# RohitMovva/VexAutonomousPlanner

Measured on AMD Instinct MI355X. Metric: trajectory sample-points/sec (batched paths), higher is better.
Workload: dtype f32; 1 GPU; c3: 4096 paths x 32 waypoints x 10000 samples per GPU; waypoints=32, samples=10000, recurrence=f64 behind fp32 rows, parallelism=paths sharded x1, no data-path collective

## Files before the change

vexautonomousplanner_amd/csrc/vap_sample.hip:

```cpp
#include "vap_device.h"
#include "vap_kernels.h"

#include <cstdio>
#include <cstdlib>
#include <type_traits>
#include <vector>

namespace vap {

static_assert(kCoefBlockDoubles == kCoefDoubles, "scratch sizing and block layout disagree");
static_assert(kGridRunBlockDoubles == kGridRunDoubles, "scratch sizing and run-table layout disagree");

template <typename OT, bool COEF_LDS, bool HI, int PPB = 1>
__global__ __launch_bounds__(kSampleThreads, 3) void k_sample(int B, int W, int S, int tile, int tiles_per_block,
                                                           const double *__restrict__ power,
                                                           const double *__restrict__ seg_rows,
                                                           const double *__restrict__ lut,
                                                           const double *__restrict__ slopes,
                                                           const double *__restrict__ meta,
                                                           const double *__restrict__ aux,
                                                           const double *__restrict__ runs,
                                                           OT *__restrict__ ox, OT *__restrict__ oy,
                                                           OT *__restrict__ oh, OT *__restrict__ ok,
                                                           OT *__restrict__ odth, double *__restrict__ ok64,
                                                           double *__restrict__ odth64, long long *__restrict__ stats)
{
    static_assert(!HI || sizeof(OT) == 4, "the fp64 side rows belong to the fp32 output mode");
    extern __shared__ __attribute__((aligned(16))) double s_coef[];
    __shared__ double sD_all[PPB * kLutN], sWt_all[PPB * kLutN];
    __shared__ double s_dx[2][kSampleThreads], s_dy[2][kSampleThreads];
    __shared__ int s_j[2][kSampleThreads];
    __shared__ OT s_th[2][kSampleThreads];
    const long long ts0 = stats ? __builtin_amdgcn_s_memtime() : 0;
    const int tid = threadIdx.x;
    const int G = W - 1;
    const int tile0 = blockIdx.x * tiles_per_block;
    if (tile0 * tile >= S) return;
    const bool writer = tile == kSampleChunk || tid < kSampleThreads - 1;
    constexpr int VW = 16 / sizeof(OT);
    const bool aligned = (S % VW) == 0;

    int p_b[PPB], p_N[PPB], p_nruns[PPB];
    bool p_live[PPB];
    double p_tmax[PPB], p_total[PPB], p_dd[PPB], p_lstep[PPB], p_tstep[PPB], p_inv[PPB], p_sk[PPB];
    double run_touch = 0.0;
#pragma unroll
    for (int pp = 0; pp < PPB; pp++) {
        const int bq = blockIdx.y * PPB + pp;
        p_live[pp] = bq < B;
        const int b = p_live[pp] ? bq : B - 1;
        p_b[pp] = b;
        const double *m = meta + (size_t)b * kMetaStride;
        p_tmax[pp] = m[0]; p_total[pp] = m[1]; p_dd[pp] = m[2];
        p_N[pp] = (int)m[3];
        const double *ax = aux + (size_t)b * kAuxStride;
        p_lstep[pp] = ax[0]; p_tstep[pp] = ax[1]; p_inv[pp] = ax[2];
        p_nruns[pp] = (int)ax[3];
        run_touch += runs[(size_t)b * kGridRunDoubles + (tid < 120 ? tid : 0)];
    }
    __shared__ double s_end[PPB][2];
    double end_d1x = 1.0, end_d1y = 1.0;
    {
        const int pp = tid < PPB ? tid : 0;
        if (seg_rows && tid < PPB && p_live[pp]) {
            end_d1x = seg_rows[((size_t)p_b[pp] * G + (G - 1)) * 12 + 6];
            end_d1y = seg_rows[((size_t)p_b[pp] * G + (G - 1)) * 12 + 7];
        }
    }
    {
        constexpr int ITER = 4;
        double vD[PPB][ITER], vW[PPB][ITER];
#pragma unroll
        for (int pp = 0; pp < PPB; pp++) {
            const bool go = p_live[pp];
#pragma unroll
            for (int it = 0; it < ITER; it++) {
                const int i = tid + it * kSampleThreads;
                vD[pp][it] = (go && i < kLutN) ? lut[(size_t)p_b[pp] * kLutN + i] : 0.0;
                vW[pp][it] = (go && slopes && i < kLutN) ? slopes[(size_t)p_b[pp] * kLutN + i] : 0.0;
            }
        }
        static_assert(ITER * kSampleThreads >= kLutN, "one pass covers the table");
#pragma unroll
        for (int pp = 0; pp < PPB; pp++) {
            if (tid == pp) {
                double rx = 1.0, ry = 1.0;
                if (fabs(end_d1x) <= 1e-9 * fabs(end_d1y) || fabs(end_d1y) <= 1e-9 * fabs(end_d1x))
                    hermite_eval_ref(seg_rows + (size_t)p_b[pp] * G * 12, p_tmax[pp], G, 1, (double)(W - 1), rx, ry);
                s_end[pp][0] = fabs(rx) <= 1e-12 * fabs(ry) ? rx : __builtin_nan("");
                s_end[pp][1] = fabs(ry) <= 1e-12 * fabs(rx) ? ry : __builtin_nan("");
            }
        }
        if constexpr (COEF_LDS) {
#pragma unroll
            for (int pp = 0; pp < PPB; pp++)
                if (p_live[pp])
                    lds_fill<4>(s_coef + (size_t)pp * G * kCoefDoubles, power + (size_t)p_b[pp] * G * kCoefDoubles, G * kCoefDoubles, tid,
                                kSampleThreads);
        }
#pragma unroll
        for (int pp = 0; pp < PPB; pp++) {
#pragma unroll
            for (int it = 0; it < ITER; it++) {
                const int i = tid + it * kSampleThreads;
                if (i < kLutN) {
                    sD_all[pp * kLutN + i] = vD[pp][it];
                    if (slopes) sWt_all[pp * kLutN + i] = vW[pp][it];
                }
            }
        }
    }
    auto grid_first_of = [&](const double *run_tab, double dd, int N, int n_runs, int kb0) {
        const int dd_exp = (__double2hiint(dd) >> 20) & 0x7ff;
        const int kf = kb0 < N - 1 ? kb0 : N - 1;
        int r = 2 + 2 * (((__double2hiint((double)kf * dd) >> 20) & 0x7ff) - dd_exp);
        r = kf <= 0 ? 0 : r < 1 ? 1 : r;
        r = r > n_runs - 1 ? n_runs - 1 : r;
        const double *e = run_tab + 3 * r;
        int ka = (int)grid_run_k0(e, 0);
        const int kb = (int)grid_run_k0(e, 1);
        double sa = e[1], da = e[2];
        if (kf < ka || kf >= kb) {
            while ((int)grid_run_k0(run_tab, r + 1) <= kf) r++;
            while (r > 0 && (int)grid_run_k0(run_tab, r) > kf) r--;
            ka = (int)grid_run_k0(run_tab, r);
            sa = run_tab[3 * r + 1];
            da = run_tab[3 * r + 2];
        }
        return sa + (double)(kf - ka) * da;
    };
#pragma unroll
    for (int pp = 0; pp < PPB; pp++)
        p_sk[pp] = (p_live[pp] && tile0 * tile < p_N[pp])
                       ? grid_first_of(runs + (size_t)p_b[pp] * kGridRunDoubles, p_dd[pp], p_N[pp], p_nruns[pp], tile0 * tile + tid * kSPT)
                       : 0.0;
    constexpr bool kSlopeOnDemand = PPB == 2;
    if (!slopes && !kSlopeOnDemand) {
        __syncthreads();
#pragma unroll
        for (int pp = 0; pp < PPB; pp++) {
            if (p_live[pp] && tile0 * tile < p_N[pp]) {
                const double *sDp = sD_all + pp * kLutN;
                for (int j = tid; j < kLutN; j += kSampleThreads) {
                    double w = 0.0;
                    if (j > 0) {
                        const double t0 = (double)(j - 1) * p_lstep[pp], t1 = (j == kLutN - 1) ? p_tmax[pp] : (double)j * p_lstep[pp];
                        w = div_inrange(t1 - t0, sDp[j] - sDp[j - 1]);
                    }
                    sWt_all[pp * kLutN + j] = w;
                }
            }
        }
    }
    __syncthreads();
    asm volatile("" ::"v"(run_touch));
    const long long ts1 = stats ? __builtin_amdgcn_s_memtime() : 0;
    const double end_param = (double)(W - 1);
    const int tab_n = W * kSamplesPerNode;
    int tiles_done = 0;

#pragma unroll 1
    for (int pp = 0; pp < PPB; pp++) {
    const int bq = blockIdx.y * PPB + pp;
    if (bq >= B) break;
    const int b = bq;
    const double *m = meta + (size_t)b * kMetaStride;
    const double t_max = m[0], total = m[1], dd = m[2];
    const int N = (int)m[3];
    const double *ax = aux + (size_t)b * kAuxStride;
    const double lstep = ax[0], tstep = ax[1], inv_tstep = ax[2];
    const int n_runs = (int)ax[3];
    const size_t row = (size_t)b * S;
    const double *sD = sD_all + pp * kLutN, *sWt = sWt_all + pp * kLutN;
    const double *pw = power + (size_t)b * G * kCoefDoubles;
    const double *coef = COEF_LDS ? s_coef + (size_t)pp * G * kCoefDoubles : pw;
    const double *run_tab = runs + (size_t)b * kGridRunDoubles;
    const double sk_first = PPB == 1 ? p_sk[0] : (pp == 0 ? p_sk[0] : p_sk[PPB - 1]);
    auto grid_first = [&](int kb0) { return grid_first_of(run_tab, dd, N, n_runs, kb0); };
    for (int tl = 0; tl < tiles_per_block; tl++) {
        const int k0 = (tile0 + tl) * tile;
        if (k0 >= S) break;
        const int kbase = k0 + tid * kSPT;
        auto store_vec = [&](OT *dst, const OT v[kSPT]) {
            if (!dst || !writer) return;
            if (aligned && kbase + kSPT <= S) {
                if constexpr (sizeof(OT) == 4) {
                    if constexpr (HI) {
                        using f4 = float __attribute__((ext_vector_type(4)));
                        f4 w = {v[0], v[1], v[2], v[3]};
                        __builtin_nontemporal_store(w, reinterpret_cast<f4 *>(dst + row + kbase));
                    } else {
                        *reinterpret_cast<float4 *>(dst + row + kbase) = make_float4(v[0], v[1], v[2], v[3]);
                    }
                } else {
                    *reinterpret_cast<double2 *>(dst + row + kbase) = make_double2(v[0], v[1]);
                    *reinterpret_cast<double2 *>(dst + row + kbase + 2) = make_double2(v[2], v[3]);
                }
            } else {
#pragma unroll
                for (int i = 0; i < kSPT; i++)
                    if (kbase + i < S) dst[row + kbase + i] = v[i];
            }
        };
        auto store_hi = [&](double *dst, const double v[kSPT]) {
            if (!writer) return;
            if ((S & 1) == 0 && kbase + kSPT <= S) {
                *reinterpret_cast<double2 *>(dst + row + kbase) = make_double2(v[0], v[1]);
                *reinterpret_cast<double2 *>(dst + row + kbase + 2) = make_double2(v[2], v[3]);
            } else {
#pragma unroll
                for (int i = 0; i < kSPT; i++)
                    if (kbase + i < S) dst[row + kbase + i] = v[i];
            }
        };
        if (k0 >= N) {
            const OT z[kSPT] = {(OT)0, (OT)0, (OT)0, (OT)0};
            store_vec(ox, z); store_vec(oy, z); store_vec(oh, z); store_vec(ok, z); store_vec(odth, z);
            if constexpr (HI) {
                const double zd[kSPT] = {0.0, 0.0, 0.0, 0.0};
                store_hi(ok64, zd); store_hi(odth64, zd);
            }
            continue;
        }
        auto tile_body = [&](auto interior_tag) {
            constexpr bool INTERIOR = decltype(interior_tag)::value;
        OT vx[kSPT], vy[kSPT], vh[kSPT], vk[kSPT], vd[kSPT];
        double vd64[HI ? kSPT : 1];
        [[maybe_unused]] double kap_even = 0.0;
        double sk = tl == 0 ? sk_first : grid_first(kbase);
        double d1x[kSPT], d1y[kSPT];
        int jjv[kSPT];
        int idx = 0;
        double tA[kSPT], sA[kSPT];
        int idxA[kSPT];
        bool redo[kSPT], any_redo = false;
        bool walk_on[kSPT], any_walk = false;
#pragma unroll
        for (int i = 0; i < kSPT; i++) {
            const int k = INTERIOR ? kbase + i : (kbase + i < N - 1 ? kbase + i : N - 1);
            if (i > 0) sk = sk + dd;
            const double s = INTERIOR ? sk : ((k == N - 1) ? total : sk);
            walk_on[i] = false;
            if (i == 0) {
                idx = lut_search_left_fixed(sD, s);
                if constexpr (!INTERIOR) idx = idx < 1 ? 1 : idx;
            } else {
                const int i1 = idx + 1 < kLutN - 1 ? idx + 1 : kLutN - 1;
                const double a0 = sD[idx], a1 = sD[i1];
                const bool st1 = idx < kLutN - 1 && a0 < s;
                const bool st2 = st1 && idx + 1 < kLutN - 1 && a1 < s;
                idx += (int)st1 + (int)st2;
                walk_on[i] = st2;
                any_walk |= st2;
            }
            sA[i] = s;
            idxA[i] = idx;
        }
        if (__builtin_expect(any_walk, 0)) {
#pragma unroll
            for (int i = 1; i < kSPT; i++) {
                if (walk_on[i]) {
                    int ix = idxA[i];
                    while (ix < kLutN - 1 && sD[ix] < sA[i]) ix++;
                    idxA[i] = ix;
                }
            }
        }
#pragma unroll
        for (int i = 0; i < kSPT; i++) {
            const double s = sA[i];
            const int idx = idxA[i];
            const double d0 = sD[idx - 1];
            const double t0 = (double)(idx - 1) * lstep;
            const bool exact = INTERIOR ? false : (s <= 0.0 || s >= total);
            double wslope;
            if (kSlopeOnDemand && !slopes) {
                const double t1 = (idx == kLutN - 1) ? t_max : (double)idx * lstep;
                wslope = div_inrange(t1 - t0, sD[idx] - d0);
            } else {
                wslope = sWt[idx];
            }
            double t = fma(wslope, s - d0, t0);
            if constexpr (!INTERIOR) t = s >= total ? end_param : t;
            bool near;
            jjv[i] = table_index_fast(t, tab_n, inv_tstep, near);
            tA[i] = t;
            redo[i] = near && !exact;
            any_redo |= redo[i];
        }
        if (__builtin_expect(any_redo, 0)) {
#pragma unroll
            for (int i = 0; i < kSPT; i++) {
                if (redo[i]) {
                    const int ix = idxA[i];
                    const double d0 = sD[ix - 1], t0 = (double)(ix - 1) * lstep;
                    const double t1 = (ix == kLutN - 1) ? t_max : (double)ix * lstep;
                    tA[i] = t0 + (t1 - t0) * (sA[i] - d0) / (sD[ix] - d0);
                    jjv[i] = table_index(tA[i], tab_n, end_param);
                }
            }
        }
#pragma unroll
        for (int i = 0; i < kSPT; i++) {
            const double t = tA[i];
            const int jj = jjv[i];
            const double tp = (jj == tab_n - 1) ? end_param : (double)jj * tstep;
            double lt;
            int sg;
            normalize_inside(tp, G, lt, sg);
            const double *c = coef + sg * kCoefDoubles;
            double ex = horner4(c + kCoefD1, lt), ey = horner4(c + kCoefD1 + 5, lt);
            if constexpr (!INTERIOR) {
                if (__builtin_expect(jj == tab_n - 1, 0)) {
                    const double rx = s_end[pp][0], ry = s_end[pp][1];
                    ex = rx == rx ? rx : ex;
                    ey = ry == ry ? ry : ey;
                }
            }
            const double fx = horner3(c + kCoefD2, lt), fy = horner3(c + kCoefD2 + 4, lt);
            const double ss = fma(ex, ex, ey * ey);
            const double num = fma(ex, fy, -(ey * fx));
            double kap;
            if constexpr (HI) {
                double kc = curvature_of(num, ss);
                asm volatile("" : "+v"(kc));
                kap = (ss >= 1e-10) ? kc : 0.0;
            } else {
                kap = (ss >= 1e-10) ? curvature_of(num, ss) : 0.0;
            }
            vk[i] = (OT)kap;
            if constexpr (HI) {
                vd64[i] = 0.0;
                if ((i & 1) == 0) {
                    kap_even = kap;
                } else if (writer) {
                    const int ke = kbase + i - 1;
                    const double v0 = (INTERIOR || ke < N) ? kap_even : 0.0, v1 = (INTERIOR || ke + 1 < N) ? kap : 0.0;
                    if (INTERIOR || ((S & 1) == 0 && ke + 2 <= S)) {
                        *reinterpret_cast<double2 *>(ok64 + row + ke) = make_double2(v0, v1);
                    } else {
                        if (ke < S) ok64[row + ke] = v0;
                        if (ke + 1 < S) ok64[row + ke + 1] = v1;
                    }
                }
            }
            vh[i] = heading_of<OT>(ey, ex);
            d1x[i] = ex;
            d1y[i] = ey;
            jjv[i] = jj;
            normalize_inside(t, G, lt, sg);
            c = coef + sg * kCoefDoubles;
            if constexpr (sizeof(OT) == 4) {
                const float *cf = reinterpret_cast<const float *>(c + kCoefPf);
                const float ltf = (float)lt;
                vx[i] = horner5f(cf, ltf);
                vy[i] = horner5f(cf + 6, ltf);
            } else {
                vx[i] = horner5(c + kCoefP, lt);
                vy[i] = horner5(c + kCoefP + 6, lt);
            }
            vd[i] = (OT)0;
        }
        const int pb = tiles_done & 1;
        tiles_done++;
        s_dx[pb][tid] = d1x[0];
        s_dy[pb][tid] = d1y[0];
        s_j[pb][tid] = jjv[0];
        s_th[pb][tid] = vh[0];
        __syncthreads();
        if (writer) {
            if constexpr (HI && sizeof(OT) == 4) {
                double dl[kSPT];
                bool act[kSPT], gen[kSPT];
                double nxv[kSPT], nyv[kSPT];
                OT nthv[kSPT];
                bool any_gen = false;
#pragma unroll
                for (int i = 0; i < kSPT; i++) {
                    const int k = kbase + i;
                    nxv[i] = (i + 1 < kSPT) ? d1x[(i + 1) % kSPT] : s_dx[pb][tid + 1];
                    nyv[i] = (i + 1 < kSPT) ? d1y[(i + 1) % kSPT] : s_dy[pb][tid + 1];
                    const int nj = (i + 1 < kSPT) ? jjv[(i + 1) % kSPT] : s_j[pb][tid + 1];
                    nthv[i] = (i + 1 < kSPT) ? vh[(i + 1) % kSPT] : s_th[pb][tid + 1];
                    act[i] = (INTERIOR || k < N - 1) && nj != jjv[i];
                    dl[i] = dtheta_f64_series(d1x[i], d1y[i], nxv[i], nyv[i], gen[i]);
                    gen[i] = gen[i] && act[i];
                    any_gen |= gen[i];
                }
                if (__builtin_expect(any_gen, 0)) {
#pragma unroll
                    for (int i = 0; i < kSPT; i++)
                        if (gen[i]) dl[i] = dtheta_f64_general(d1x[i], d1y[i], nxv[i], nyv[i]);
                }
#pragma unroll
                for (int i = 0; i < kSPT; i++) {
                    const double v = dtheta_f64_wrap(dl[i], vh[i], nthv[i]);
                    vd64[i] = act[i] ? v : vd64[i];
                    vd[i] = (INTERIOR || kbase + i < N - 1) ? (OT)vd64[i] : vd[i];
                }
            } else {
#pragma unroll
            for (int i = 0; i < kSPT; i++) {
                const int k = kbase + i;
                if (INTERIOR || k < N - 1) {
                    const double nx = (i + 1 < kSPT) ? d1x[(i + 1) % kSPT] : s_dx[pb][tid + 1];
                    const double ny = (i + 1 < kSPT) ? d1y[(i + 1) % kSPT] : s_dy[pb][tid + 1];
                    const int nj = (i + 1 < kSPT) ? jjv[(i + 1) % kSPT] : s_j[pb][tid + 1];
                    const OT nth = (i + 1 < kSPT) ? vh[(i + 1) % kSPT] : s_th[pb][tid + 1];
                    if constexpr (sizeof(OT) == 8) {
                        vd[i] = fabs(nth - vh[i]);
                    } else if constexpr (HI) {
                        if (nj != jjv[i]) vd64[i] = dtheta_f64(d1x[i], d1y[i], nx, ny, vh[i], nth);
                        vd[i] = (OT)vd64[i];
                    } else {
                        if (nj != jjv[i]) vd[i] = dtheta_f32(d1x[i], d1y[i], nx, ny, vh[i], nth);
                    }
                }
            }
            }
            if (!INTERIOR && k0 + kSampleChunk > N) {
#pragma unroll
                for (int i = 0; i < kSPT; i++)
                    if (kbase + i >= N) {
                        vx[i] = vy[i] = vh[i] = vk[i] = vd[i] = (OT)0;
                        if constexpr (HI) vd64[i] = 0.0;
                    }
            }
            store_vec(ox, vx); store_vec(oy, vy); store_vec(oh, vh); store_vec(ok, vk);
            if constexpr (HI) store_hi(odth64, vd64);
            store_vec(odth, vd);
        }
            };
        const bool interior = k0 > 0 && k0 + kSampleThreads * kSPT < N - 1 && aligned && (S & 1) == 0 && k0 + kSampleThreads * kSPT <= S;
        if (interior) tile_body(std::true_type{});
        else tile_body(std::false_type{});
    }
    }
    if (stats && (tid & 63) == 0) {
        long long *st = stats + ((size_t)(blockIdx.y * gridDim.x + blockIdx.x) * 4 + (tid >> 6)) * 4;
        st[0] = ts1 - ts0;
        st[1] = __builtin_amdgcn_s_memtime() - ts1;
        st[2] = 0;
        st[3] = 0;
    }
}

hipError_t launch_sample(hipStream_t st, bool f64, int B, int W, int S, const double *pw, const double *lut,
                         const double *slopes, const double *meta, const double *aux, const double *runs, void *x,
                         void *y, void *h, void *k, void *dth, double *k64, double *dth64, const double *seg)
{
    const bool hi = !f64 && k64 && dth64;
    const int tile = S <= kSampleChunk ? kSampleChunk : kSampleTile;
    const int n_tiles = (S + tile - 1) / tile;
    int split = (2048 + B - 1) / B;
    split = split < 1 ? 1 : (split > n_tiles ? n_tiles : split);
    const int tiles_per_block = (n_tiles + split - 1) / split;
    const bool in_lds = (W - 1) <= kLdsCoefSegments;
    const int ppb = (n_tiles == 1 && B >= 8192 && in_lds && (W - 1) <= 16) ? 2 : 1;
    const dim3 grid((n_tiles + tiles_per_block - 1) / tiles_per_block, (B + ppb - 1) / ppb);
    const size_t lds = in_lds ? sizeof(double) * (size_t)ppb * (W - 1) * kCoefDoubles : 0;
    static const bool want_stats = getenv("VAP_SAMPLE_STATS") != nullptr;
    long long *stats = nullptr;
    const size_t n_waves = (size_t)grid.x * grid.y * 4;
    if (want_stats) (void)hipMalloc(&stats, n_waves * 4 * sizeof(long long));
#define VAP_SAMPLE(OT_, LDS_, HI_, PPB_)                                                                            \
    hipLaunchKernelGGL((k_sample<OT_, LDS_, HI_, PPB_>), grid, dim3(kSampleThreads), lds, st, B, W, S, tile, tiles_per_block, pw, seg, lut, \
                       slopes, meta, aux, runs, (OT_ *)x, (OT_ *)y, (OT_ *)h, (OT_ *)k, (OT_ *)dth, k64, dth64, stats)
    if (ppb == 2) {
        if (f64) VAP_SAMPLE(double, true, false, 2);
        else if (hi) VAP_SAMPLE(float, true, true, 2);
        else VAP_SAMPLE(float, true, false, 2);
    } else if (f64) { if (in_lds) VAP_SAMPLE(double, true, false, 1); else VAP_SAMPLE(double, false, false, 1); }
    else if (hi) { if (in_lds) VAP_SAMPLE(float, true, true, 1); else VAP_SAMPLE(float, false, true, 1); }
    else { if (in_lds) VAP_SAMPLE(float, true, false, 1); else VAP_SAMPLE(float, false, false, 1); }
#undef VAP_SAMPLE
    if (stats) {
        std::vector<long long> h(n_waves * 4);
        (void)hipStreamSynchronize(st);
        (void)hipMemcpy(h.data(), stats, h.size() * sizeof(long long), hipMemcpyDeviceToHost);
        (void)hipFree(stats);
        double sum[4] = {0, 0, 0, 0};
        for (size_t w = 0; w < n_waves; w++)
            for (int k = 0; k < 4; k++) sum[k] += (double)h[w * 4 + k];
        fprintf(stderr, "[sample grid %ux%u, %d tiles/block] per-wave mean ticks: stage %.0f tiles %.0f\n", grid.x,
                grid.y, tiles_per_block, sum[0] / n_waves, sum[1] / n_waves);
    }
    return hipGetLastError();
}

}
```

Measured before the change: 46.06 billion sample-points/s.

## Split per-thread sample phases into halves and pack neighbour LDS exchange

For the fp32-with-fp64-side-rows mode, each thread now processes its samples in two halves, computing the heading-delta for the first half's interior pairs before the barrier. This is meant to cut live register pressure, so the launch bound rises to 4 waves per SIMD. The four neighbour arrays are merged into one padded struct array in LDS. Alignment is now checked on the host, including base-pointer alignment, and passed as bits. Stats instrumentation is compiled out unless a macro is defined. The fp32 delta row is now written only when its pointer is non-null. The cost is more template instantiations, and the higher occupancy target may force register spills.

```diff
diff --git a/vexautonomousplanner_amd/csrc/vap_sample.hip b/vexautonomousplanner_amd/csrc/vap_sample.hip
--- a/vexautonomousplanner_amd/csrc/vap_sample.hip
+++ b/vexautonomousplanner_amd/csrc/vap_sample.hip
@@ -1,6 +1,7 @@
 #include "vap_device.h"
 #include "vap_kernels.h"
 
+#include <cstdint>
 #include <cstdio>
 #include <cstdlib>
 #include <type_traits>
@@ -11,8 +12,14 @@
 static_assert(kCoefBlockDoubles == kCoefDoubles, "scratch sizing and block layout disagree");
 static_assert(kGridRunBlockDoubles == kGridRunDoubles, "scratch sizing and run-table layout disagree");
 
-template <typename OT, bool COEF_LDS, bool HI, int PPB = 1>
-__global__ __launch_bounds__(kSampleThreads, 3) void k_sample(int B, int W, int S, int tile, int tiles_per_block,
+constexpr int k_sample_waves(int halves, int ppb) { return halves == 2 && ppb == 1 ? 4 : 3; }
+#ifdef VAP_SAMPLE_STATS
+#define VAP_STATS_PARAM , long long *__restrict__ stats
+#else
+#define VAP_STATS_PARAM
+#endif
+template <typename OT, bool COEF_LDS, bool HI, int PPB = 1, int HALVES = 1>
+__global__ __launch_bounds__(kSampleThreads, k_sample_waves(HALVES, PPB)) void k_sample(int B, int W, int S, int tile, int tiles_per_block, int align_bits,
                                                            const double *__restrict__ power,
                                                            const double *__restrict__ seg_rows,
                                                            const double *__restrict__ lut,
@@ -23,22 +30,24 @@
                                                            OT *__restrict__ ox, OT *__restrict__ oy,
                                                            OT *__restrict__ oh, OT *__restrict__ ok,
                                                            OT *__restrict__ odth, double *__restrict__ ok64,
-                                                           double *__restrict__ odth64, long long *__restrict__ stats)
+                                                           double *__restrict__ odth64 VAP_STATS_PARAM)
 {
+    static_assert(HALVES == 1 || HALVES == 2, "a thread's samples go through the phases all at once or in two halves");
     static_assert(!HI || sizeof(OT) == 4, "the fp64 side rows belong to the fp32 output mode");
     extern __shared__ __attribute__((aligned(16))) double s_coef[];
     __shared__ double sD_all[PPB * kLutN], sWt_all[PPB * kLutN];
-    __shared__ double s_dx[2][kSampleThreads], s_dy[2][kSampleThreads];
-    __shared__ int s_j[2][kSampleThreads];
-    __shared__ OT s_th[2][kSampleThreads];
+    struct Neighbour { double dx, dy; OT th; int j; };
+    __shared__ Neighbour s_nb[2][kSampleThreads + 1];
+#ifdef VAP_SAMPLE_STATS
     const long long ts0 = stats ? __builtin_amdgcn_s_memtime() : 0;
+#endif
     const int tid = threadIdx.x;
     const int G = W - 1;
     const int tile0 = blockIdx.x * tiles_per_block;
     if (tile0 * tile >= S) return;
     const bool writer = tile == kSampleChunk || tid < kSampleThreads - 1;
-    constexpr int VW = 16 / sizeof(OT);
-    const bool aligned = (S % VW) == 0;
+    const bool aligned = (align_bits & 1) != 0;
+    const bool aligned_hi = (align_bits & 2) != 0;
 
     int p_b[PPB], p_N[PPB], p_nruns[PPB];
     bool p_live[PPB];
@@ -154,7 +163,9 @@
     }
     __syncthreads();
     asm volatile("" ::"v"(run_touch));
+#ifdef VAP_SAMPLE_STATS
     const long long ts1 = stats ? __builtin_amdgcn_s_memtime() : 0;
+#endif
     const double end_param = (double)(W - 1);
     const int tab_n = W * kSamplesPerNode;
     int tiles_done = 0;
@@ -204,7 +215,7 @@
         };
         auto store_hi = [&](double *dst, const double v[kSPT]) {
             if (!writer) return;
-            if ((S & 1) == 0 && kbase + kSPT <= S) {
+            if (aligned_hi && kbase + kSPT <= S) {
                 *reinterpret_cast<double2 *>(dst + row + kbase) = make_double2(v[0], v[1]);
                 *reinterpret_cast<double2 *>(dst + row + kbase + 2) = make_double2(v[2], v[3]);
             } else {
@@ -224,6 +235,7 @@
         }
         auto tile_body = [&](auto interior_tag) {
             constexpr bool INTERIOR = decltype(interior_tag)::value;
+        constexpr int HS = kSPT / HALVES;
         OT vx[kSPT], vy[kSPT], vh[kSPT], vk[kSPT], vd[kSPT];
         double vd64[HI ? kSPT : 1];
         [[maybe_unused]] double kap_even = 0.0;
@@ -231,17 +243,76 @@
         double d1x[kSPT], d1y[kSPT];
         int jjv[kSPT];
         int idx = 0;
-        double tA[kSPT], sA[kSPT];
-        int idxA[kSPT];
-        bool redo[kSPT], any_redo = false;
-        bool walk_on[kSPT], any_walk = false;
-#pragma unroll
-        for (int i = 0; i < kSPT; i++) {
-            const int k = INTERIOR ? kbase + i : (kbase + i < N - 1 ? kbase + i : N - 1);
-            if (i > 0) sk = sk + dd;
+        const int pb = tiles_done & 1;
+        tiles_done++;
+        auto dtheta_range = [&](auto ga_tag, auto gb_tag) {
+            constexpr int GA = decltype(ga_tag)::value, GB = decltype(gb_tag)::value, GN = GB - GA + 1;
+            if constexpr (HI && sizeof(OT) == 4) {
+                double dl[GN];
+                bool act[GN], gen[GN];
+                double nxv[GN], nyv[GN];
+                OT nthv[GN];
+                bool any_gen = false;
+#pragma unroll
+                for (int q = 0; q < GN; q++) {
+                    const int i = GA + q;
+                    const int k = kbase + i;
+                    nxv[q] = (i + 1 < kSPT) ? d1x[(i + 1) % kSPT] : s_nb[pb][tid + 1].dx;
+                    nyv[q] = (i + 1 < kSPT) ? d1y[(i + 1) % kSPT] : s_nb[pb][tid + 1].dy;
+                    const int nj = (i + 1 < kSPT) ? jjv[(i + 1) % kSPT] : s_nb[pb][tid + 1].j;
+                    nthv[q] = (i + 1 < kSPT) ? vh[(i + 1) % kSPT] : s_nb[pb][tid + 1].th;
+                    act[q] = (INTERIOR || k < N - 1) && nj != jjv[i];
+                    dl[q] = dtheta_f64_series(d1x[i], d1y[i], nxv[q], nyv[q], gen[q]);
+                    gen[q] = gen[q] && act[q];
+                    any_gen |= gen[q];
+                }
+                if (__builtin_expect(any_gen, 0)) {
+#pragma unroll
+                    for (int q = 0; q < GN; q++)
+                        if (gen[q]) dl[q] = dtheta_f64_general(d1x[GA + q], d1y[GA + q], nxv[q], nyv[q]);
+                }
+#pragma unroll
+                for (int q = 0; q < GN; q++) {
+                    const int i = GA + q;
+                    const double v = dtheta_f64_wrap(dl[q], vh[i], nthv[q]);
+                    vd64[i] = act[q] ? v : vd64[i];
+                }
+            } else {
+#pragma unroll
+                for (int i = GA; i <= GB; i++) {
+                    const int k = kbase + i;
+                    if (INTERIOR || k < N - 1) {
+                        const double nx = (i + 1 < kSPT) ? d1x[(i + 1) % kSPT] : s_nb[pb][tid + 1].dx;
+                        const double ny = (i + 1 < kSPT) ? d1y[(i + 1) % kSPT] : s_nb[pb][tid + 1].dy;
+                        const int nj = (i + 1 < kSPT) ? jjv[(i + 1) % kSPT] : s_nb[pb][tid + 1].j;
+                        const OT nth = (i + 1 < kSPT) ? vh[(i + 1) % kSPT] : s_nb[pb][tid + 1].th;
+                        if constexpr (sizeof(OT) == 8) {
+                            vd[i] = fabs(nth - vh[i]);
+                        } else if constexpr (HI) {
+                            if (nj != jjv[i]) vd64[i] = dtheta_f64(d1x[i], d1y[i], nx, ny, vh[i], nth);
+                            vd[i] = (OT)vd64[i];
+                        } else {
+                            if (nj != jjv[i]) vd[i] = dtheta_f32(d1x[i], d1y[i], nx, ny, vh[i], nth);
+                        }
+                    }
+                }
+            }
+        };
+#pragma unroll
+        for (int h = 0; h < HALVES; h++) {
+        const int g0 = h * HS;
+        double tA[HS], sA[HS];
+        int idxA[HS];
+        bool redo[HS], any_redo = false;
+        bool walk_on[HS], any_walk = false;
+#pragma unroll
+        for (int i = 0; i < HS; i++) {
+            const int g = g0 + i;
+            const int k = INTERIOR ? kbase + g : (kbase + g < N - 1 ? kbase + g : N - 1);
+            if (g > 0) sk = sk + dd;
             const double s = INTERIOR ? sk : ((k == N - 1) ? total : sk);
             walk_on[i] = false;
-            if (i == 0) {
+            if (g == 0) {
                 idx = lut_search_left_fixed(sD, s);
                 if constexpr (!INTERIOR) idx = idx < 1 ? 1 : idx;
             } else {
@@ -258,7 +329,7 @@
         }
         if (__builtin_expect(any_walk, 0)) {
 #pragma unroll
-            for (int i = 1; i < kSPT; i++) {
+            for (int i = (g0 == 0 ? 1 : 0); i < HS; i++) {
                 if (walk_on[i]) {
                     int ix = idxA[i];
                     while (ix < kLutN - 1 && sD[ix] < sA[i]) ix++;
@@ -266,8 +337,9 @@
                 }
             }
         }
-#pragma unroll
-        for (int i = 0; i < kSPT; i++) {
+        if constexpr (HALVES > 1) idx = idxA[HS - 1];
+#pragma unroll
+        for (int i = 0; i < HS; i++) {
             const double s = sA[i];
             const int idx = idxA[i];
             const double d0 = sD[idx - 1];
@@ -283,26 +355,27 @@
             double t = fma(wslope, s - d0, t0);
             if constexpr (!INTERIOR) t = s >= total ? end_param : t;
             bool near;
-            jjv[i] = table_index_fast(t, tab_n, inv_tstep, near);
+            jjv[g0 + i] = table_index_fast(t, tab_n, inv_tstep, near);
             tA[i] = t;
             redo[i] = near && !exact;
             any_redo |= redo[i];
         }
         if (__builtin_expect(any_redo, 0)) {
 #pragma unroll
-            for (int i = 0; i < kSPT; i++) {
+            for (int i = 0; i < HS; i++) {
                 if (redo[i]) {
                     const int ix = idxA[i];
                     const double d0 = sD[ix - 1], t0 = (double)(ix - 1) * lstep;
                     const double t1 = (ix == kLutN - 1) ? t_max : (double)ix * lstep;
                     tA[i] = t0 + (t1 - t0) * (sA[i] - d0) / (sD[ix] - d0);
-                    jjv[i] = table_index(tA[i], tab_n, end_param);
-                }
-            }
-        }
-#pragma unroll
-        for (int i = 0; i < kSPT; i++) {
-            const double t = tA[i];
+                    jjv[g0 + i] = table_index(tA[i], tab_n, end_param);
+                }
+            }
+        }
+#pragma unroll
+        for (int q = 0; q < HS; q++) {
+            const int i = g0 + q;
+            const double t = tA[q];
             const int jj = jjv[i];
             const double tp = (jj == tab_n - 1) ? end_param : (double)jj * tstep;
             double lt;
@@ -336,7 +409,7 @@
                 } else if (writer) {
                     const int ke = kbase + i - 1;
                     const double v0 = (INTERIOR || ke < N) ? kap_even : 0.0, v1 = (INTERIOR || ke + 1 < N) ? kap : 0.0;
-                    if (INTERIOR || ((S & 1) == 0 && ke + 2 <= S)) {
+                    if (INTERIOR || (aligned_hi && ke + 2 <= S)) {
                         *reinterpret_cast<double2 *>(ok64 + row + ke) = make_double2(v0, v1);
                     } else {
                         if (ke < S) ok64[row + ke] = v0;
@@ -347,7 +420,6 @@
             vh[i] = heading_of<OT>(ey, ex);
             d1x[i] = ex;
             d1y[i] = ey;
-            jjv[i] = jj;
             normalize_inside(t, G, lt, sg);
             c = coef + sg * kCoefDoubles;
             if constexpr (sizeof(OT) == 4) {
@@ -355,69 +427,27 @@
                 const float ltf = (float)lt;
                 vx[i] = horner5f(cf, ltf);
                 vy[i] = horner5f(cf + 6, ltf);
+                asm volatile("" : "+v"(vx[i]), "+v"(vy[i]));
             } else {
                 vx[i] = horner5(c + kCoefP, lt);
                 vy[i] = horner5(c + kCoefP + 6, lt);
             }
             vd[i] = (OT)0;
         }
-        const int pb = tiles_done & 1;
-        tiles_done++;
-        s_dx[pb][tid] = d1x[0];
-        s_dy[pb][tid] = d1y[0];
-        s_j[pb][tid] = jjv[0];
-        s_th[pb][tid] = vh[0];
+        if (h == 0) {
+            Neighbour *nb = &s_nb[pb][tid];
+            nb->dx = d1x[0];
+            nb->dy = d1y[0];
+            nb->j = jjv[0];
+            nb->th = vh[0];
+        }
+        if constexpr (HALVES == 2) {
+            if (h == 0) dtheta_range(std::integral_constant<int, 0>{}, std::integral_constant<int, HS - 2>{});
+        }
+        }
         __syncthreads();
         if (writer) {
-            if constexpr (HI && sizeof(OT) == 4) {
-                double dl[kSPT];
-                bool act[kSPT], gen[kSPT];
-                double nxv[kSPT], nyv[kSPT];
-                OT nthv[kSPT];
-                bool any_gen = false;
-#pragma unroll
-                for (int i = 0; i < kSPT; i++) {
-                    const int k = kbase + i;
-                    nxv[i] = (i + 1 < kSPT) ? d1x[(i + 1) % kSPT] : s_dx[pb][tid + 1];
-                    nyv[i] = (i + 1 < kSPT) ? d1y[(i + 1) % kSPT] : s_dy[pb][tid + 1];
-                    const int nj = (i + 1 < kSPT) ? jjv[(i + 1) % kSPT] : s_j[pb][tid + 1];
-                    nthv[i] = (i + 1 < kSPT) ? vh[(i + 1) % kSPT] : s_th[pb][tid + 1];
-                    act[i] = (INTERIOR || k < N - 1) && nj != jjv[i];
-                    dl[i] = dtheta_f64_series(d1x[i], d1y[i], nxv[i], nyv[i], gen[i]);
-                    gen[i] = gen[i] && act[i];
-                    any_gen |= gen[i];
-                }
-                if (__builtin_expect(any_gen, 0)) {
-#pragma unroll
-                    for (int i = 0; i < kSPT; i++)
-                        if (gen[i]) dl[i] = dtheta_f64_general(d1x[i], d1y[i], nxv[i], nyv[i]);
-                }
-#pragma unroll
-                for (int i = 0; i < kSPT; i++) {
-                    const double v = dtheta_f64_wrap(dl[i], vh[i], nthv[i]);
-                    vd64[i] = act[i] ? v : vd64[i];
-                    vd[i] = (INTERIOR || kbase + i < N - 1) ? (OT)vd64[i] : vd[i];
-                }
-            } else {
-#pragma unroll
-            for (int i = 0; i < kSPT; i++) {
-                const int k = kbase + i;
-                if (INTERIOR || k < N - 1) {
-                    const double nx = (i + 1 < kSPT) ? d1x[(i + 1) % kSPT] : s_dx[pb][tid + 1];
-                    const double ny = (i + 1 < kSPT) ? d1y[(i + 1) % kSPT] : s_dy[pb][tid + 1];
-                    const int nj = (i + 1 < kSPT) ? jjv[(i + 1) % kSPT] : s_j[pb][tid + 1];
-                    const OT nth = (i + 1 < kSPT) ? vh[(i + 1) % kSPT] : s_th[pb][tid + 1];
-                    if constexpr (sizeof(OT) == 8) {
-                        vd[i] = fabs(nth - vh[i]);
-                    } else if constexpr (HI) {
-                        if (nj != jjv[i]) vd64[i] = dtheta_f64(d1x[i], d1y[i], nx, ny, vh[i], nth);
-                        vd[i] = (OT)vd64[i];
-                    } else {
-                        if (nj != jjv[i]) vd[i] = dtheta_f32(d1x[i], d1y[i], nx, ny, vh[i], nth);
-                    }
-                }
-            }
-            }
+            dtheta_range(std::integral_constant<int, (HALVES == 2 ? HS - 1 : 0)>{}, std::integral_constant<int, kSPT - 1>{});
             if (!INTERIOR && k0 + kSampleChunk > N) {
 #pragma unroll
                 for (int i = 0; i < kSPT; i++)
@@ -428,14 +458,23 @@
             }
             store_vec(ox, vx); store_vec(oy, vy); store_vec(oh, vh); store_vec(ok, vk);
             if constexpr (HI) store_hi(odth64, vd64);
-            store_vec(odth, vd);
+            if constexpr (HI && sizeof(OT) == 4) {
+                if (odth) {
+#pragma unroll
+                    for (int i = 0; i < kSPT; i++) vd[i] = (OT)vd64[i];
+                    store_vec(odth, vd);
+                }
+            } else {
+                store_vec(odth, vd);
+            }
         }
             };
-        const bool interior = k0 > 0 && k0 + kSampleThreads * kSPT < N - 1 && aligned && (S & 1) == 0 && k0 + kSampleThreads * kSPT <= S;
+        const bool interior = k0 > 0 && k0 + kSampleThreads * kSPT < N - 1 && aligned && aligned_hi && k0 + kSampleThreads * kSPT <= S;
         if (interior) tile_body(std::true_type{});
         else tile_body(std::false_type{});
     }
     }
+#ifdef VAP_SAMPLE_STATS
     if (stats && (tid & 63) == 0) {
         long long *st = stats + ((size_t)(blockIdx.y * gridDim.x + blockIdx.x) * 4 + (tid >> 6)) * 4;
         st[0] = ts1 - ts0;
@@ -443,6 +482,7 @@
         st[2] = 0;
         st[3] = 0;
     }
+#endif
 }
 
 hipError_t launch_sample(hipStream_t st, bool f64, int B, int W, int S, const double *pw, const double *lut,
@@ -459,21 +499,33 @@
     const int ppb = (n_tiles == 1 && B >= 8192 && in_lds && (W - 1) <= 16) ? 2 : 1;
     const dim3 grid((n_tiles + tiles_per_block - 1) / tiles_per_block, (B + ppb - 1) / ppb);
     const size_t lds = in_lds ? sizeof(double) * (size_t)ppb * (W - 1) * kCoefDoubles : 0;
+    const size_t vw = f64 ? 2 : 4;
+    const uintptr_t bases = (uintptr_t)x | (uintptr_t)y | (uintptr_t)h | (uintptr_t)k | (uintptr_t)dth;
+    const uintptr_t bases_hi = (uintptr_t)k64 | (uintptr_t)dth64;
+    const int align_bits = (((size_t)S % vw) == 0 && (bases & 15) == 0 ? 1 : 0) | ((S & 1) == 0 && (bases_hi & 15) == 0 ? 2 : 0);
+#ifdef VAP_SAMPLE_STATS
     static const bool want_stats = getenv("VAP_SAMPLE_STATS") != nullptr;
     long long *stats = nullptr;
     const size_t n_waves = (size_t)grid.x * grid.y * 4;
     if (want_stats) (void)hipMalloc(&stats, n_waves * 4 * sizeof(long long));
-#define VAP_SAMPLE(OT_, LDS_, HI_, PPB_)                                                                            \
-    hipLaunchKernelGGL((k_sample<OT_, LDS_, HI_, PPB_>), grid, dim3(kSampleThreads), lds, st, B, W, S, tile, tiles_per_block, pw, seg, lut, \
-                       slopes, meta, aux, runs, (OT_ *)x, (OT_ *)y, (OT_ *)h, (OT_ *)k, (OT_ *)dth, k64, dth64, stats)
+#define VAP_STATS_ARG , stats
+#else
+#define VAP_STATS_ARG
+#endif
+#define VAP_SAMPLE(OT_, LDS_, HI_, PPB_, HALVES_)                                                                   \
+    hipLaunchKernelGGL((k_sample<OT_, LDS_, HI_, PPB_, HALVES_>), grid, dim3(kSampleThreads), lds, st, B, W, S, tile, tiles_per_block, \
+                       align_bits, pw, seg, lut, slopes, meta, aux, runs, (OT_ *)x, (OT_ *)y, (OT_ *)h, (OT_ *)k, (OT_ *)dth, k64,   \
+                       dth64 VAP_STATS_ARG)
     if (ppb == 2) {
-        if (f64) VAP_SAMPLE(double, true, false, 2);
-        else if (hi) VAP_SAMPLE(float, true, true, 2);
-        else VAP_SAMPLE(float, true, false, 2);
-    } else if (f64) { if (in_lds) VAP_SAMPLE(double, true, false, 1); else VAP_SAMPLE(double, false, false, 1); }
-    else if (hi) { if (in_lds) VAP_SAMPLE(float, true, true, 1); else VAP_SAMPLE(float, false, true, 1); }
-    else { if (in_lds) VAP_SAMPLE(float, true, false, 1); else VAP_SAMPLE(float, false, false, 1); }
+        if (f64) VAP_SAMPLE(double, true, false, 2, 1);
+        else if (hi) VAP_SAMPLE(float, true, true, 2, 2);
+        else VAP_SAMPLE(float, true, false, 2, 1);
+    } else if (f64) { if (in_lds) VAP_SAMPLE(double, true, false, 1, 1); else VAP_SAMPLE(double, false, false, 1, 1); }
+    else if (hi) { if (in_lds) VAP_SAMPLE(float, true, true, 1, 2); else VAP_SAMPLE(float, false, true, 1, 2); }
+    else { if (in_lds) VAP_SAMPLE(float, true, false, 1, 1); else VAP_SAMPLE(float, false, false, 1, 1); }
 #undef VAP_SAMPLE
+#undef VAP_STATS_ARG
+#ifdef VAP_SAMPLE_STATS
     if (stats) {
         std::vector<long long> h(n_waves * 4);
         (void)hipStreamSynchronize(st);
@@ -485,6 +537,7 @@
         fprintf(stderr, "[sample grid %ux%u, %d tiles/block] per-wave mean ticks: stage %.0f tiles %.0f\n", grid.x,
                 grid.y, tiles_per_block, sum[0] / n_waves, sum[1] / n_waves);
     }
+#endif
     return hipGetLastError();
 }
 
```

After: 47.22 billion sample-points/s, median of 6. 1.03x the previous value.
